# ProjectTorreyPines/TorJ.jl

Measured on AMD Instinct MI355X. Metric: ray-steps/sec, 1e5-ray EC fan on 1 MI355X (+ 2/4/8-GPU scaling), higher is better.
Workload: dtype f64

## Files before the change

### include/torj_hip.h

```cpp
#ifndef TORJ_HIP_H
#define TORJ_HIP_H

#include <stdint.h>

#ifdef __cplusplus
extern "C" {
#endif

#define TORJ_ABI_VERSION 8

enum torj_status {
    TORJ_RAY_OK = 0,
    TORJ_RAY_LEFT_PLASMA = 1,
    TORJ_RAY_ABSORBED = 2,
    TORJ_RAY_NAN = 3,
    TORJ_RAY_REFLECTED = 4,
    TORJ_RAY_ENTRY_FAIL = 5,
    TORJ_RAY_MAX_STEPS = 6
};

typedef struct torj_plasma_s *torj_plasma_t;

int torj_abi_version(void);
const char *torj_build_id(void);
// ... 224 lines not shown
                    int *steps, double *dP_shell, double *P_dep, double *traj, int n_gpus,
                    int n_shards);

typedef struct {
    int n;
    const double *x0, *N0;
    const double *weights;
    const double *psi_grid;
    const double *x_launch, *s0;
    double *state;
    int *status, *steps;
    double *dP_shell;
    double *P_dep;
    double *traj;
    uint64_t *counters;
} torj_beam_shard;
int torj_trace_beam_device(torj_plasma_t p, const torj_trace_cfg *cfg, int n_gpus, int n_psi,
                           const torj_beam_shard *shards);

int torj_set_sched(torj_plasma_t p, int mode, int waves);

int torj_trace_check(torj_plasma_t p, void *stream);

int torj_timing(torj_plasma_t p, int enable);
int torj_timing_read(torj_plasma_t p, int *calls, double *trace_ms, double *post_ms);

int torj_beam_timing_read(torj_plasma_t p, int n_gpus, int *calls, double *trace_ms, double *post_ms,
                          double *reduce_ms);

int torj_beam_comm_info(torj_plasma_t p, int n_gpus, int *device, int *nranks, int *rank);

int torj_power_deposition_profile(torj_plasma_t p, int n_rays, const int *n_points, const double *s,
                                  const double *x, const double *dP_ds, int n_psi,
                                  const double *psi_dP_dV, double *dP_dV, double *P);

int torj_shell_volumes(torj_plasma_t p, int n_psi, const double *psi_grid, double *dV);

#ifdef __cplusplus
}
#endif
#endif
```

### torj.jl_amd/csrc/torj_fitdepo.hpp

```cpp
#pragma once
#include "torj_math.hpp"

namespace torj {

constexpr int kSmpBlk = 64;
TORJ_HD size_t smp_at(size_t j, int i, size_t rows) {
    return ((size_t)((unsigned)i / kSmpBlk) * rows + j) * kSmpBlk + (unsigned)i % kSmpBlk;
}
TORJ_HD size_t smp_elems(size_t n, size_t rows) { return (n + kSmpBlk - 1) / kSmpBlk * kSmpBlk * rows; }

struct FitArgs {
    const double *coef;
    Grid g;
    int n, n_psi;
    double ds;
    const double *grid;
    const double *w;
    const double *x_launch;
    const double *s0;
    const int *steps;
    const double *smp_psi, *smp_dpds, *smp_s;
    size_t rows;
    int s_uniform;
    double *E, *Gpsi, *GP;
    int *cnt;
    double *Fopen;
    double *dPs;
    int *kstar;
    double *dP;
    double *Pray;
    const int *npts;
};

TORJ_HD int imin(int x, int y) { return x < y ? x : y; }
TORJ_HD int imax(int x, int y) { return x > y ? x : y; }

constexpr int kChunk = 8;
constexpr int kWalkChunk = 4;
constexpr int kWalkChunkStream = 1;

struct RayData {
    const FitArgs *a;
    int i, m;
    double s0, psiL;
    TORJ_HD double S(int j) const {
        if (a->npts) return a->smp_s[smp_at(j, i, a->rows)];
        if (j == 0) return 0.0;
        return a->s_uniform ? fma((double)(j - 1), a->ds, s0) : a->smp_s[smp_at(j - 1, i, a->rows)];
    }
    TORJ_HD double h(int j) const { return (j == 0 && !a->npts) ? s0 : S(j + 1) - S(j); }
    TORJ_HD double Ypsi(int j) const {
        if (a->npts) return a->smp_psi[smp_at(j, i, a->rows)];
        return j == 0 ? psiL : a->smp_psi[smp_at(j - 1, i, a->rows)];
    }
// ... 145 lines not shown
    bool spilled;
    int run_k0, run_k1, run_d;
    int runs, last_d;
    TORJ_HD void init() {
#pragma unroll
        for (int u = 0; u < NC; u++) oq[u] = -1, oF[u] = 0.0;
        spilled = false;
        run_d = 0, run_k0 = run_k1 = 0;
        runs = 0, last_d = 0;
    }
    TORJ_HD void piece(int d) {
        if (d != last_d) runs++, last_d = d;
    }
    TORJ_HD void cadd(int k, int v) {
        __hip_atomic_fetch_add(a->cnt + (size_t)k * a->n + i, v, __ATOMIC_RELAXED, __HIP_MEMORY_SCOPE_AGENT);
    }
    TORJ_HD void flush_run() {
        if (run_d == 0) return;
        const int lo = run_k0 < run_k1 ? run_k0 : run_k1, hi = run_k0 < run_k1 ? run_k1 : run_k0;
        cadd(lo, 1);
        cadd(hi + 1, -1);
        run_d = 0;
    }
    TORJ_HD void close(int q, double d) {
        double *p = a->dPs + (size_t)q * a->n + i;
        __hip_atomic_fetch_add(p, d, __ATOMIC_RELAXED, __HIP_MEMORY_SCOPE_AGENT);
    }
    TORJ_HD void toggle(int q, double Fr) {
        bool hit = false;
        double fo = 0.0;
#pragma unroll
        for (int u = 0; u < NC; u++)
            if (!hit && oq[u] == q) hit = true, fo = oF[u], oq[u] = -1;
        if (!hit && spilled) {
            double &m = a->Fopen[(size_t)q * a->n + i];
            fo = m;
            if (!isnan(fo)) hit = true, m = NAN;
        }
        if (hit) {
            close(q, fabs(Fr - fo));
            return;
        }
        bool placed = false;
#pragma unroll
        for (int u = 0; u < NC; u++)
            if (!placed && oq[u] < 0) placed = true, oq[u] = q, oF[u] = Fr;
        if (!placed) {
            a->Fopen[(size_t)oq[0] * a->n + i] = oF[0];
            spilled = true;
            oq[0] = q, oF[0] = Fr;
        }
    }
    TORJ_HD void root(int k, double Fr, int d) {
        if constexpr (CAP) {
            int &c = a->cnt[(size_t)k * a->n + i];
            if (c >= kMaxRoots) return;
            c++;
        } else if (d == run_d && k == run_k1 + d) {
            run_k1 = k;
        } else {
            flush_run();
            run_d = d, run_k0 = run_k1 = k;
        }
        if (k - 1 >= 0 && k - 1 <= a->n_psi - 2) toggle(k - 1, Fr);
        if (k <= a->n_psi - 2) toggle(k, Fr);
    }
};

template <class W_>
TORJ_HD void walk_segment(W_ &W, const Cubic &qs, double y1, const Cubic &qP, bool first) {
    const FitArgs &a = *W.a;
    const double A = 3.0 * qs.d, B = 2.0 * qs.c, C = qs.b;
    const double disc = B * B - 4.0 * A * C;
    double c1 = qs.h, c2 = qs.h;
    const double dh = fma(fma(A, qs.h, B), qs.h, C);
    const double tv = -B * A;
    const bool keep = (C > 0.0 && dh > 0.0) || (C < 0.0 && dh < 0.0);
    const bool vout = A == 0.0 || tv <= 0.0 || tv >= 2.0 * A * A * qs.h;
    if (!(keep && vout) && (A != 0.0 ? disc > 0.0 : B != 0.0)) {
        double r1 = NAN, r2 = NAN;
        if (A != 0.0) {
            const double sq = sqrt(disc);
            const double qq = -0.5 * (B + (B >= 0.0 ? sq : -sq));
            r1 = qq / A;
            if (qq != 0.0) r2 = C / qq;
        } else {
            r1 = -C / B;
        }
// ... 177 lines not shown
}

template <int NC>
TORJ_HD void fit_depo_ray(const FitArgs &a, int i, double psiL) {
    const int m = a.npts ? a.npts[i] : a.steps[i] + 2;
    if (m < 4 || (!a.npts && !(a.s0[i] > 0.0))) {
        a.kstar[i] = a.n_psi;
        a.Pray[i] = 0.0;
        return;
    }
    RayData R{&a, i, m, a.npts ? 0.0 : a.s0[i], psiL};
    nak_eliminate(R);
    Walker<NC> W{&a, i, 0.0, 0.0, Cursor{&a, 0, 0.0, 0.0}};
    W.init();
    walk_ray(W, R);
    fit_depo_finish(a, i, R, W);
}

#ifndef TORJ_DEPO_Q
#define TORJ_DEPO_Q 64
#endif
constexpr int kDepoQ = TORJ_DEPO_Q, kDepoW = 32;
enum { kDsFhi, kDsFlo, kDsOF0, kDsOF1, kDsMl, kDsMr, kDsMn, kDsMPl, kDsMPr, kDsMPn, kDsYl, kDsPl, kDsNd };
enum { kDsJ, kDsC, kDsOQ0, kDsOQ1, kDsSpill, kDsRk0, kDsRk1, kDsRd, kDsRuns, kDsLast, kDsNi };
struct DepoStream {
    double *d;
    int *v;
};
static_assert(kOpenCache == 2, "DepoStream holds two open-shell slots");

TORJ_HD bool depo_load(const DepoStream &ds, size_t n, int i, Walker<kOpenCache> &W, WalkCarry &C) {
    const int j = ds.v[kDsJ * n + i];
    if (j < 0) return false;
    const double *d = ds.d + i;
    const int *v = ds.v + i;
    W.Fhi = d[kDsFhi * n], W.Flo = d[kDsFlo * n];
    W.oF[0] = d[kDsOF0 * n], W.oF[1] = d[kDsOF1 * n];
    C.Ml = d[kDsMl * n], C.Mr = d[kDsMr * n], C.Mn = d[kDsMn * n];
    C.MPl = d[kDsMPl * n], C.MPr = d[kDsMPr * n], C.MPn = d[kDsMPn * n];
    C.yl = d[kDsYl * n], C.Pl = d[kDsPl * n];
    C.j = j;
    W.cur.c = v[kDsC * n];
    W.cur.load();
    W.oq[0] = v[kDsOQ0 * n], W.oq[1] = v[kDsOQ1 * n];
    W.spilled = v[kDsSpill * n] != 0;
    W.run_k0 = v[kDsRk0 * n], W.run_k1 = v[kDsRk1 * n], W.run_d = v[kDsRd * n];
    W.runs = v[kDsRuns * n], W.last_d = v[kDsLast * n];
    return true;
}
TORJ_HD void depo_save(const DepoStream &ds, size_t n, int i, const Walker<kOpenCache> &W, const WalkCarry &C) {
    double *d = ds.d + i;
    int *v = ds.v + i;
    d[kDsFhi * n] = W.Fhi, d[kDsFlo * n] = W.Flo;
    d[kDsOF0 * n] = W.oF[0], d[kDsOF1 * n] = W.oF[1];
    d[kDsMl * n] = C.Ml, d[kDsMr * n] = C.Mr, d[kDsMn * n] = C.Mn;
    d[kDsMPl * n] = C.MPl, d[kDsMPr * n] = C.MPr, d[kDsMPn * n] = C.MPn;
    d[kDsYl * n] = C.yl, d[kDsPl * n] = C.Pl;
    v[kDsC * n] = W.cur.c;
    v[kDsOQ0 * n] = W.oq[0], v[kDsOQ1 * n] = W.oq[1];
    v[kDsSpill * n] = W.spilled ? 1 : 0;
    v[kDsRk0 * n] = W.run_k0, v[kDsRk1 * n] = W.run_k1, v[kDsRd * n] = W.run_d;
    v[kDsRuns * n] = W.runs, v[kDsLast * n] = W.last_d;
    v[kDsJ * n] = C.j;
}

TORJ_HD bool depo_windows(const RayData &R, Walker<kOpenCache> &W, WalkCarry &C, bool started, int last) {
    for (;;) {
        const int ja = started ? C.j : 0, jb = ja + kDepoQ, r0 = jb + 2 + kDepoW;
        if (r0 + 1 > last) break;
        nak_eliminate_rows(R, started ? ja + 3 : 1, r0);
        if (!started) {
            walk_start(W, R, C);
            started = true;
        }
        walk_segments(W, R, C, jb);
    }
    return started;
}

TORJ_HD void fit_depo_stream(const FitArgs &a, const DepoStream &ds, int i, double psiL, int S) {
    if (!(a.s0[i] > 0.0)) return;
    const int j = ds.v[kDsJ * (size_t)a.n + i];
    if ((j < 0 ? 0 : j) + kDepoQ + 3 + kDepoW > S) return;
    RayData R{&a, i, S + 2, a.s0[i], psiL};
    Walker<kOpenCache> W{&a, i, 0.0, 0.0, Cursor{&a, 0, 0.0, 0.0}};
    W.init();
    WalkCarry C{};
    const bool started = depo_load(ds, a.n, i, W, C);
    if (depo_windows(R, W, C, started, S)) depo_save(ds, a.n, i, W, C);
}

TORJ_HD bool depo_next_window(const DepoStream &ds, size_t n, int i, int S, int &ja, bool &started) {
    const int j = ds.v[kDsJ * n + i];
    started = j >= 0;
    ja = started ? j : 0;
    return ja + kDepoQ + 3 + kDepoW <= S;
}
TORJ_HD void fit_depo_stream_elim(const FitArgs &a, const DepoStream &ds, int i, double psiL, int S) {
    if (!(a.s0[i] > 0.0)) return;
    int ja;
    bool started;
    if (!depo_next_window(ds, a.n, i, S, ja, started)) return;
    RayData R{&a, i, S + 2, a.s0[i], psiL};
    nak_eliminate_rows(R, started ? ja + 3 : 1, ja + kDepoQ + 2 + kDepoW);
}
TORJ_HD void fit_depo_stream_walk(const FitArgs &a, const DepoStream &ds, int i, double psiL, int S) {
    if (!(a.s0[i] > 0.0)) return;
    int ja;
    bool started;
    if (!depo_next_window(ds, a.n, i, S, ja, started)) return;
    RayData R{&a, i, S + 2, a.s0[i], psiL};
    Walker<kOpenCache> W{&a, i, 0.0, 0.0, Cursor{&a, 0, 0.0, 0.0}};
    W.init();
    WalkCarry C{};
    if (started)
        depo_load(ds, a.n, i, W, C);
    else
        walk_start(W, R, C);
    walk_segments<kWalkChunkStream>(W, R, C, ja + kDepoQ);
    depo_save(ds, a.n, i, W, C);
}

TORJ_HD void fit_depo_tail(const FitArgs &a, const DepoStream &ds, int i, double psiL) {
    const int m = a.steps[i] + 2;
    if (m < 4 || !(a.s0[i] > 0.0)) {
        a.kstar[i] = a.n_psi;
        a.Pray[i] = 0.0;
        return;
    }
    RayData R{&a, i, m, a.s0[i], psiL};
    Walker<kOpenCache> W{&a, i, 0.0, 0.0, Cursor{&a, 0, 0.0, 0.0}};
    W.init();
    WalkCarry C{};
    bool started = depo_load(ds, a.n, i, W, C);
    started = depo_windows(R, W, C, started, m - 2);
    nak_eliminate_rows(R, started ? C.j + 3 : 1, m - 2);
    if (!started) walk_start(W, R, C);
// ... 6 lines not shown
```

### torj.jl_amd/csrc/torj_hip.hip

```cpp
#include <hip/hip_runtime.h>

#include <algorithm>
#include <cmath>
#include <cstring>
#include <mutex>
#include <vector>

#include "../../include/torj_hip.h"
#include "torj_math.hpp"
#include "torj_entry.hpp"
#include "torj_fitdepo.hpp"
#include "torj_warm.hpp"

using namespace torj;

#include "torj_host_util.hpp"
#include "torj_args.hpp"
#include "torj_k_fused.hpp"
#include "torj_k_traj.hpp"
#include "torj_k_alpha.hpp"
#include "torj_k_scan.hpp"
#include "torj_k_depo.hpp"
#include "torj_k_points.hpp"
#include "torj_k_beams.hpp"
// ... 573 lines not shown
        if (p->stage.h_pinned)
            (void)hipHostFree(p->stage.h);
        else
            free(p->stage.h);
    }
    for (int r = 0; r < 2; r++) {
        if (p->stage.up[r]) (void)hipEventDestroy(p->stage.up[r]);
        if (p->stage.tr[r]) (void)hipEventDestroy(p->stage.tr[r]);
        if (p->stage.dn[r]) (void)hipEventDestroy(p->stage.dn[r]);
    }
    if (p->stage.sc) (void)hipStreamDestroy(p->stage.sc);
    if (p->d_coef) (void)hipFree(p->d_coef);
    if (p->d_cellp) (void)hipFree(p->d_cellp);
    if (p->stream) (void)hipStreamDestroy(p->stream);
    if (p->ev_Nin) (void)hipEventDestroy(p->ev_Nin);
    if (p->ev_Nout) (void)hipEventDestroy(p->ev_Nout);
    if (p->ev_U) (void)hipEventDestroy(p->ev_U);
    if (p->ev_B) (void)hipEventDestroy(p->ev_B);
    if (p->cbuild.d) (void)hipFree(p->cbuild.d);
    if (p->d_psi) (void)hipFree(p->d_psi);
    if (p->sched.d) (void)hipFree(p->sched.d);
    if (p->fit.d) (void)hipFree(p->fit.d);
    if (p->d_flags) (void)hipFree(p->d_flags);
    if (p->chunk.d) (void)hipFree(p->chunk.d);
    for (hipEvent_t e : p->ev_pool) (void)hipEventDestroy(e);
    if (p->ws.d) (void)hipFree(p->ws.d);
    if (p->beams.d) (void)hipFree(p->beams.d);
    if (p->mk.d) (void)hipFree(p->mk.d);
    if (p->split.d) (void)hipFree(p->split.d);
    if (p->batch.d) (void)hipFree(p->batch.d);
    for (int q = 0; q < torj_plasma_s::kRing; q++) {
        if (p->ev_T[q]) (void)hipEventDestroy(p->ev_T[q]);
        if (p->ev_A[q]) (void)hipEventDestroy(p->ev_A[q]);
        if (p->ev_S[q]) (void)hipEventDestroy(p->ev_S[q]);
    }
    if (p->ev_J) (void)hipEventDestroy(p->ev_J);
    if (p->ev_F) (void)hipEventDestroy(p->ev_F);
    if (p->ev_D) (void)hipEventDestroy(p->ev_D);
    if (p->stream2) (void)hipStreamDestroy(p->stream2);
    if (p->streamT) (void)hipStreamDestroy(p->streamT);
    if (p->streamS) (void)hipStreamDestroy(p->streamS);
    if (p->streamD) (void)hipStreamDestroy(p->streamD);
    delete p;
    return 0;
}

// ... 947 lines not shown
    if (!out && reduce) {
        std::vector<double *> d_dP(n_gpus);
        for (int k = 0; k < n_gpus; k++) d_dP[k] = shards[k].dP_shell;
        out = beam_reduce(p, n_gpus, d_dP, n_psi, same);
    }
    (void)hipSetDevice(p->device);
    return out;
}

int torj_trace_check(torj_plasma_t p, void *stream) {
    if (!p) return fail("bad plasma handle");
    if (!p->d_flags) return 0;
    HIPCK(hipSetDevice(p->device));
    HIPCK(hipStreamSynchronize((hipStream_t)stream));
    int flags = 0;
    HIPCK(hipMemcpy(&flags, p->d_flags, sizeof(int), hipMemcpyDeviceToHost));
    if (flags) HIPCK(hipMemset(p->d_flags, 0, sizeof(int)));
    if (flags & 1) return fail("psi_dP_dV must be strictly increasing");
    if (flags & 2) return fail("work-queue watchdog fired (ready-queue stalled)");
    if (flags & 4) return fail("work queue did not retire every ray group");
    return 0;
}

}
```

### torj.jl_amd/csrc/torj_k_depo.hpp

```cpp
#pragma once
#include "torj_args.hpp"
#include "torj_fitdepo.hpp"

constexpr int kFitGridLds = 4096;

__global__ void __launch_bounds__(64, 2) k_fit_depo(FitArgs a) {
    extern __shared__ double s_grid[];
    if (a.n_psi <= kFitGridLds) {
        for (int k = threadIdx.x; k < a.n_psi; k += 64) s_grid[k] = a.grid[k];
        __syncthreads();
        a.grid = s_grid;
    }
    const int i = blockIdx.x * 64 + threadIdx.x;
    if (i >= a.n) return;
    const double xl[3] = {a.x_launch[i], a.x_launch[a.n + i], a.x_launch[2 * a.n + i]};
    fit_depo_ray<kOpenCache>(a, i, psi_at(a.coef, a.g, xl));
}
__device__ __forceinline__ bool fit_grid_lds(FitArgs &a) {
    extern __shared__ double s_grid[];
    if (a.n_psi > kFitGridLds) return false;
    for (int k = threadIdx.x; k < a.n_psi; k += 64) s_grid[k] = a.grid[k];
    __syncthreads();
    a.grid = s_grid;
    return true;
// ... 21 lines not shown
    fit_depo_stream(a, ds, i, psiL, S);
}
#ifndef TORJ_DEPO_ELIM_WAVES
#define TORJ_DEPO_ELIM_WAVES 4
#endif
__global__ void __launch_bounds__(64, TORJ_DEPO_ELIM_WAVES) k_depo_elim(FitArgs a, DepoStream ds, const int *sinfo,
                                                                        int s_cap) {
    const int i = blockIdx.x * 64 + threadIdx.x;
    int S;
    double psiL;
    if (i >= a.n || !depo_stream_gate(a, ds, sinfo, s_cap, i, S, psiL)) return;
    fit_depo_stream_elim(a, ds, i, psiL, S);
}
#ifndef TORJ_DEPO_WALK_WAVES
#define TORJ_DEPO_WALK_WAVES 3
#endif
__global__ void __launch_bounds__(64, TORJ_DEPO_WALK_WAVES) k_depo_walk(FitArgs a, DepoStream ds, const int *sinfo,
                                                                        int s_cap) {
    fit_grid_lds(a);
    const int i = blockIdx.x * 64 + threadIdx.x;
    int S;
    double psiL;
    if (i >= a.n || !depo_stream_gate(a, ds, sinfo, s_cap, i, S, psiL)) return;
    fit_depo_stream_walk(a, ds, i, psiL, S);
}
__global__ void __launch_bounds__(64, 2) k_depo_tail(FitArgs a, DepoStream ds) {
    fit_grid_lds(a);
    const int i = blockIdx.x * 64 + threadIdx.x;
    if (i >= a.n) return;
    const double xl[3] = {a.x_launch[i], a.x_launch[a.n + i], a.x_launch[2 * a.n + i]};
    fit_depo_tail(a, ds, i, psi_at(a.coef, a.g, xl));
}
__global__ void __launch_bounds__(64) k_profile_samples(FitArgs a, const long *off, const double *s,
                                                        const double *x, size_t n_all, const double *dpds) {
    const int i = blockIdx.x * 64 + threadIdx.x;
    if (i >= a.n) return;
    for (int j = 0; j < a.npts[i]; j++) {
        const size_t q = (size_t)off[i] + j;
        const double xq[3] = {x[q], x[n_all + q], x[2 * n_all + q]};
        const size_t o = smp_at(j, i, a.rows);
        const_cast<double *>(a.smp_psi)[o] = psi_at(a.coef, a.g, xq);
        const_cast<double *>(a.smp_dpds)[o] = dpds[q];
        const_cast<double *>(a.smp_s)[o] = s[q];
    }
}
__global__ void __launch_bounds__(64, 2) k_fit_profile(FitArgs a) {
    extern __shared__ double s_grid[];
// ... 48 lines not shown
```

### torj.jl_amd/csrc/torj_plasma.hpp

```cpp
#pragma once
#include <rccl/rccl.h>

#include <algorithm>
#include <mutex>
#include <vector>

#include "torj_args.hpp"
#include "torj_host_util.hpp"
#include "torj_math.hpp"

static void bspl1d_prefilter(int n, const double *y, size_t ystride, double *c, size_t cstride) {
    auto C = [&](int k) -> double & { return c[(size_t)k * cstride]; };
    auto Y = [&](int k) { return y[(size_t)k * ystride]; };
    C(1) = Y(0);
    C(n) = Y(n - 1);
    const int m = n - 2;
    if (m > 0) {
        std::vector<double> cp(m), dp(m);
        for (int k = 0; k < m; k++) {
            double r = 6.0 * Y(k + 1);
            if (k == 0) r -= C(1);
            if (k == m - 1) r -= C(n);
            const double den = 4.0 - (k > 0 ? cp[k - 1] : 0.0);
            cp[k] = 1.0 / den;
// ... 94 lines not shown
    std::vector<double> coef;
    std::vector<double> psi_nodes;
    double *d_coef = nullptr;
    double *d_cellp = nullptr;
    int n_vol = 0;
    double v1 = 0, vn = 0;
    std::vector<double> vol_coef;
    double psi_prof_max = 0;
    hipStream_t stream = nullptr;
    GrowBuf sched;
    int sched_mode = -1, sched_waves = 0;
    int lanes_per_ray = 0;
    GrowBuf chunk;
    GrowBuf fit;
    bool timing = false;
    int timing_calls = 0;
    GrowBuf batch;
    std::vector<hipEvent_t> ev_pool;
    size_t ev_used = 0;
    GrowBuf ws;
    GrowBuf beams;
    GrowBuf mk;
    int *d_flags = nullptr;
    int n_cu = 256;
    std::mutex mu;
    std::vector<torj_plasma_s *> replicas;
    std::vector<ncclComm_t> comms;
    struct BeamStage {
        void *d = nullptr, *h = nullptr;
        size_t d_cap = 0, h_cap = 0;
        bool h_pinned = false;
        hipStream_t sc = nullptr;
        hipEvent_t up[2] = {}, tr[2] = {}, dn[2] = {};
    } stage;
    double reduce_ms = 0.0;
    int reduce_calls = 0;
    GrowBuf split;
    hipStream_t stream2 = nullptr, streamT = nullptr;
    hipStream_t streamS = nullptr;
    hipStream_t streamD = nullptr;
    static constexpr int kRing = kSplitRing;
    hipEvent_t ev_T[kRing] = {}, ev_A[kRing] = {}, ev_S[kRing] = {}, ev_J = nullptr, ev_F = nullptr;
    hipEvent_t ev_D = nullptr;
    hipEvent_t ev_Nin = nullptr, ev_Nout = nullptr;
    hipEvent_t ev_U = nullptr;
    GrowBuf cbuild;
// ... 34 lines not shown
    return 0;
}

static int ensure_device(torj_plasma_s *p) {
    std::lock_guard<std::mutex> lk(p->mu);
    int ndev = 0;
    HIPCK(hipGetDeviceCount(&ndev));
    if (p->device < 0 || p->device >= ndev)
        return fail("device %d not available (%d HIP devices)", p->device, ndev);
    HIPCK(hipSetDevice(p->device));
    if (p->d_flags) return 0;
    if (p->d_coef) return fail("handle's device state is incomplete (an earlier initialisation failed)");
    HIPCK(hipMalloc(&p->d_coef, p->coef.size() * sizeof(double)));
    HIPCK(hipMemcpy(p->d_coef, p->coef.data(), p->coef.size() * sizeof(double),
                    hipMemcpyHostToDevice));
    {
        std::vector<double> cp((size_t)(p->g.nR - 1) * (p->g.nZ - 1) * kCellRec);
        cell_power_table(p->coef.data(), p->g.nR, p->g.nZ, p->g.hR, p->g.hZ, cp.data());
        HIPCK(hipMalloc(&p->d_cellp, cp.size() * sizeof(double)));
        HIPCK(hipMemcpy(p->d_cellp, cp.data(), cp.size() * sizeof(double), hipMemcpyHostToDevice));
    }
    HIPCK(hipStreamCreateWithFlags(&p->stream, hipStreamNonBlocking));
    HIPCK(hipDeviceGetAttribute(&p->n_cu, hipDeviceAttributeMultiprocessorCount, p->device));
    int *flags = nullptr;
    HIPCK(hipMalloc(&flags, sizeof(int)));
    if (hipMemset(flags, 0, sizeof(int)) != hipSuccess) {
        (void)hipFree(flags);
        return fail("hipMemset of the launch flags failed");
    }
    p->d_flags = flags;
    return 0;
}

static int ensure_buf(torj_plasma_s *p, GrowBuf &b, size_t bytes) {
    std::lock_guard<std::mutex> lk(p->mu);
    return b.reserve(bytes);
}

static int mirror_sync(torj_plasma_s *p) {
    std::lock_guard<std::mutex> lk(p->mu);
    if (!p->coef_stale && !p->psi_stale) return 0;
    HIPCK(hipSetDevice(p->device));
    HIPCK(hipEventSynchronize(p->ev_B));
    if (p->coef_stale) {
        HIPCK(hipMemcpy(p->coef.data(), p->d_coef, p->coef.size() * sizeof(double), hipMemcpyDeviceToHost));
        p->coef_stale = false;
// ... 78 lines not shown
```

### torj.jl_amd/csrc/torj_split.hpp

```cpp
#pragma once
#include <algorithm>
#include <atomic>

#include "torj_args.hpp"
#include "torj_fitdepo.hpp"
#include "torj_host_util.hpp"
#ifndef TORJ_SPLIT_PLAN_ONLY
#include "torj_dispatch.hpp"
#include "torj_k_alpha.hpp"
#include "torj_k_depo.hpp"
#include "torj_k_scan.hpp"
#include "torj_k_traj.hpp"
#include "torj_plasma.hpp"

static size_t fit_grid_lds(int n_psi) { return n_psi <= kFitGridLds ? (size_t)n_psi * sizeof(double) : 0; }

static int fit_zero(const FitArgs &fa, hipStream_t st) {
    const size_t L = (size_t)fa.n_psi, N = (size_t)fa.n;
    HIPCK(hipMemsetAsync(fa.cnt, 0, (L + 1) * N * sizeof(int), st));
    HIPCK(hipMemsetAsync(fa.Fopen, 0xFF, L * N * sizeof(double), st));
    HIPCK(hipMemsetAsync(fa.dPs, 0, L * N * sizeof(double), st));
    return 0;
}
#endif
// ... 127 lines not shown
    sp.tx = (double *)take(6 * pl.b_n8);
    sp.stau = (double *)take(pl.b_n8);
    sp.spsi = (double *)take(pl.b_n8);
    sp.sPdep = (double *)take(pl.b_n8);
    sp.tinfo = (int *)take(pl.b_n4);
    sp.sinfo = (int *)take(pl.b_n4);
    sp.defer = pl.b_defer ? (unsigned long long *)take(pl.b_defer) : nullptr;
    rg.dcnt = pl.b_dcnt ? (unsigned *)take(pl.b_dcnt) : nullptr;
    if (pl.dstream) {
        rg.ds.d = (double *)take(pl.b_dsd);
        rg.ds.v = (int *)take(pl.b_dsi);
    }
}

#ifndef TORJ_SPLIT_PLAN_ONLY
static int split_plan(SplitPlan &pl, const torj_plasma_s *p, const TraceArgs &a, int DM, bool walk,
                      bool negl_skip) {
    size_t free_b = 0, total_b = 0;
    HIPCK(hipMemGetInfo(&free_b, &total_b));
    split_plan_sizes(pl, p->sched_mode, p->sched_waves, free_b, a, DM, walk, negl_skip);
    return 0;
}

static int split_trace(torj_plasma_s *p, TraceArgs a, int DM, bool tr, hipStream_t s, const FitArgs *fa,
                       DepoStream *dso, bool negl_skip, double tiny_alpha) {
    SplitPlan pl;
    if (split_plan(pl, p, a, DM, fa && dso, negl_skip)) return -1;
    constexpr int R = SplitPlan::R;
    const size_t n = pl.n;
    if (ensure_split(p, pl.bytes)) return -1;
    SplitArgs sp{};
    SplitRing rg;
    split_carve(pl, (char *)p->split.d, sp, rg);
    const DepoStream ds = rg.ds;
    if (dso) *dso = ds;
    sp.nf = pl.nf;
    sp.tile_cap = pl.tile_cap;
    sp.tile_margin = pl.tile_margin;
    sp.nan_step = pl.nan_step;
    sp.zval = 0.0;
    sp.defer_lrm = pl.defer_lrm;
    sp.zlatch = pl.zlatch;
    sp.tiny_alpha = split_tiny_alpha(pl, a, tiny_alpha);
    sp.tval = 0.0;
    const int tflag_nan_from = env_has("TORJ_TEST_TFLAG_NAN") ? std::max(0, env_int("TORJ_TEST_TFLAG_NAN", 0)) : -1;
    if (tflag_nan_from >= 0) {
        static std::atomic<bool> warned{false};
        if (!warned.exchange(true))
            fprintf(stderr, "libtorj_hip: TORJ_TEST_TFLAG_NAN is set -- a TEST HOOK: alpha waves fully "
                            "flagged by the tiny_alpha proof write NaN\n");
    }

    const bool serial = pl.serial, dstream = pl.dstream;
    static const bool scan_own = env_int("TORJ_SPLIT_SCAN", 1) != 0;
    hipStream_t sT = serial ? s : p->streamT, s2 = serial ? s : p->stream2;
    hipStream_t s3 = serial ? s : (scan_own ? p->streamS : p->stream2);
    const bool depo_own = dstream && (pl.dstream_env == 2 || pl.dstream_env == 4) && !serial;
    const bool depo_traj = dstream && pl.dstream_env == 5 && !serial;
    if (depo_own && !p->streamD) {
        int lo = 0, hi = 0;
        HIPCK(hipDeviceGetStreamPriorityRange(&lo, &hi));
        HIPCK(hipStreamCreateWithPriority(&p->streamD, hipStreamNonBlocking, stream_prio("TORJ_DEPO_PRIO", lo, lo, hi)));
    }
    hipStream_t sD = depo_own ? p->streamD : s3;
    if (!serial) {
        HIPCK(hipEventRecord(p->ev_F, s));
        HIPCK(hipStreamWaitEvent(sT, p->ev_F, 0));
        HIPCK(hipStreamWaitEvent(s2, p->ev_F, 0));
        if (s3 != s2) HIPCK(hipStreamWaitEvent(s3, p->ev_F, 0));
    }
    HIPCK(hipMemsetAsync(sp.stau, 0, 3 * pl.b_n8, sT));
    HIPCK(hipMemsetAsync(sp.sinfo, 0, pl.b_n4, sT));
    if (dstream) HIPCK(hipMemsetAsync(ds.v + kDsJ * n, 0xFF, n * sizeof(int), sT));
    if (rg.dcnt) HIPCK(hipMemsetAsync(rg.dcnt, 0, pl.n_blk * sizeof(unsigned), s2));
    if (fa && fit_zero(*fa, s3)) return -1;
    const size_t fit_lds = fa ? fit_grid_lds(fa->n_psi) : 0;
    const int G = (int)((n + 63) / 64);
    const size_t lds_bytes = pl.traj_lds_bytes;
    const bool lds_traj = pl.traj_mode == kTrajLds;
    const bool tile_traj = pl.traj_mode == kTrajTile, cell_traj = pl.traj_mode == kTrajCell;
    sp.traj_mode = pl.traj_mode;
    const int wpb = std::min(8, std::max(1, (G + p->n_cu - 1) / p->n_cu));
    const int n_blocks = pl.n_blk;
    auto depo_pair = [&](hipStream_t st, int cap) {
        hipLaunchKernelGGL(k_depo_elim, dim3(G), dim3(64), 0, st, *fa, ds, sp.sinfo, cap);
        hipLaunchKernelGGL(k_depo_walk, dim3(G), dim3(64), fit_lds, st, *fa, ds, sp.sinfo, cap);
    };
    for (int b = 0; b < n_blocks; b++) {
        sp.k0 = pl.block_k0(b);
        sp.kb = pl.block_len(b);
        const int r = b % R;
        sp.ain = rg.ain[r];
        sp.psib = rg.psib[r];
        sp.zflag = rg.zflags[r];
        sp.gflag = rg.gflags[r];
        sp.zval = (pl.zflag_nan_from >= 0 && sp.k0 >= pl.zflag_nan_from) ? NAN : 0.0;
        sp.tval = (tflag_nan_from >= 0 && sp.k0 >= tflag_nan_from) ? NAN : 0.0;
        sp.alpha = rg.alphas[r];
        sp.awork = pl.b_awork ? rg.aworks[r] : nullptr;
        if (b >= R) HIPCK(hipStreamWaitEvent(sT, p->ev_S[r], 0));
        if (depo_traj && b >= pl.depo_lag) {
            const int bw = b - pl.depo_lag;
            HIPCK(hipStreamWaitEvent(sT, p->ev_S[bw % R], 0));
            depo_pair(sT, pl.window_cap(bw));
        }
        with_depo_traj(DM, tr, [&](auto D, auto T) {
            if (cell_traj)
                hipLaunchKernelGGL((k_traj_cell<D(), T()>), dim3(G), dim3(64), 0, sT, a, sp);
            else if (tile_traj)
// ... 81 lines not shown
```

### torj.jl_amd/torj_hip/_lib.py

```python
from __future__ import annotations

import ctypes as C
import os
import subprocess

import numpy as np

_PKG = os.path.dirname(os.path.abspath(__file__))
_ROOT = os.path.dirname(_PKG)
LIB_PATH = os.environ.get("TORJ_HIP_LIB") or os.path.join(_ROOT, "build", "libtorj_hip.so")
CSRC = os.path.join(_ROOT, "csrc")

_dp = C.POINTER(C.c_double)
_ip = C.POINTER(C.c_int)
_u64p = C.POINTER(C.c_uint64)
_hp = C.POINTER(C.c_void_p)


class TorjError(RuntimeError):
    pass


class TraceCfg(C.Structure):
    _fields_ = [("omega", C.c_double), ("mode", C.c_int), ("ds", C.c_double),
# ... 69 lines not shown
    "torj_abs_albajar_fast": (C.c_int, [C.c_int, _dp, _dp, _dp, _dp, _dp, _dp, C.c_int, _dp]),
    "torj_alpha_warm": (C.c_int, [C.c_int] + [_dp] * 7 + [C.c_int, C.c_int, _dp, _dp]),
    "torj_refractive_index_sq": (C.c_int, [C.c_int, _dp, _dp, _dp, C.c_int, _dp]),
    "torj_pol_tor_angles_2_vector": (None, [C.c_double, C.c_double, _dp]),
    "torj_launch_peripheral_rays": (C.c_int, [_dp, _dp, C.c_double, C.c_double, C.c_double,
                                              C.c_int, C.c_int, C.c_int, _ip, _dp, _dp, _dp]),
    "torj_ray_entry": (C.c_int, [C.c_void_p, C.c_int, _dp, _dp, C.c_double, C.c_int, _dp, _dp,
                                 _dp, _ip]),
    "torj_ray_entry_device": (C.c_int, [C.c_void_p, C.c_int, C.c_void_p, C.c_void_p, C.c_double,
                                        C.c_int, C.c_void_p, C.c_void_p, C.c_void_p, C.c_void_p,
                                        C.c_void_p]),
    "torj_ray_entry_gpu": (C.c_int, [C.c_void_p, C.c_int, _dp, _dp, C.c_double, C.c_int, _dp,
                                     _dp, _dp, _ip]),
    "torj_trace": (C.c_int, [C.c_void_p, C.POINTER(TraceCfg), C.c_int, _dp, _dp, _dp, C.c_int,
                             _dp, _dp, _ip, _ip, _dp, _dp, _dp]),
    "torj_trace_ex": (C.c_int, [C.c_void_p, C.POINTER(TraceCfg), C.c_int, _dp, _dp, _dp, C.c_int,
                                _dp, _dp, _dp, _dp, _ip, _ip, _dp, _dp, _dp]),
    "torj_trace_beam": (C.c_int, [C.c_void_p, C.POINTER(TraceCfg), C.c_int, _dp, _dp, _dp, C.c_int,
                                  _dp, _dp, _dp, _dp, _ip, _ip, _dp, _dp, _dp, C.c_int, C.c_int]),
    "torj_trace_beam_device": (C.c_int, [C.c_void_p, C.POINTER(TraceCfg), C.c_int, C.c_int,
                                         C.POINTER(BeamShard)]),
    "torj_set_sched": (C.c_int, [C.c_void_p, C.c_int, C.c_int]),
    "torj_trace_check": (C.c_int, [C.c_void_p, C.c_void_p]),
    "torj_timing": (C.c_int, [C.c_void_p, C.c_int]),
    "torj_timing_read": (C.c_int, [C.c_void_p, _ip, _dp, _dp]),
    "torj_beam_timing_read": (C.c_int, [C.c_void_p, C.c_int, _ip, _dp, _dp, _dp]),
    "torj_beam_comm_info": (C.c_int, [C.c_void_p, C.c_int, _ip, _ip, _ip]),
    "torj_trace_device": (C.c_int, [C.c_void_p, C.POINTER(TraceCfg), C.c_int, C.c_void_p,
                                    C.c_void_p, C.c_void_p, C.c_int, C.c_void_p, C.c_void_p,
                                    C.c_void_p, C.c_void_p, C.c_void_p, C.c_void_p, C.c_void_p,
                                    C.c_void_p, C.c_void_p]),
    "torj_trace_device_ex": (C.c_int, [C.c_void_p, C.POINTER(TraceCfg), C.c_int] +
                             [C.c_void_p] * 3 + [C.c_int] + [C.c_void_p] * 11),
    "torj_trace_beams_device": (C.c_int, [C.c_void_p, C.POINTER(TraceCfg), C.c_int, _ip, _dp, _ip] +
                                [C.c_void_p] * 3 + [C.c_int] + [C.c_void_p] * 11),
    "torj_trace_beams": (C.c_int, [C.c_void_p, C.POINTER(TraceCfg), C.c_int, _ip, _dp, _ip, _dp, _dp,
                                   _dp, C.c_int, _dp, _dp, _dp, _dp, _ip, _ip, _dp, _dp, _dp]),
    "torj_ray_entry_beams_device": (C.c_int, [C.c_void_p, C.c_int, _ip, _dp, _ip] + [C.c_void_p] * 7),
    "torj_ray_entry_beams_gpu": (C.c_int, [C.c_void_p, C.c_int, _ip, _dp, _ip, _dp, _dp, _dp, _dp, _dp,
                                           _ip]),
    "torj_trace_beams_plasmas_device": (C.c_int, [C.c_void_p, C.c_int, _hp, _ip, C.POINTER(TraceCfg), C.c_int,
                                                  _ip, _dp, _ip] + [C.c_void_p] * 3 + [C.c_int] +
                                        [C.c_void_p] * 11),
    "torj_trace_beams_plasmas": (C.c_int, [C.c_void_p, C.c_int, _hp, _ip, C.POINTER(TraceCfg), C.c_int, _ip, _dp,
                                           _ip, _dp, _dp, _dp, C.c_int, _dp, _dp, _dp, _dp, _ip, _ip, _dp, _dp,
                                           _dp]),
# ... 74 lines not shown
```

### torj.jl_amd/torj_hip/plasma.py

```python
from __future__ import annotations

import ctypes as C

import numpy as np

from ._lib import check, dptr, f64, lib, soa

FIELDS = ("psi", "lnne", "lnTe", "Br", "Bz", "Bphi")


class Plasma:

    def __init__(self, R_coords, Z_coords, psi_norm_data, psi_prof, ne_prof, Te_prof, Br_data,
                 Bz_data, Bphi_data, eqt1d_psi_norm, eqt1d_volume, device: int = 0):
        R, Z = f64(R_coords), f64(Z_coords)
        nR, nZ = len(R), len(Z)

        def m(a):
            a = np.asarray(a, dtype=np.float64)
            if a.shape != (nR, nZ):
                raise ValueError(f"2-D map has shape {a.shape}, expected {(nR, nZ)}")
            return np.ascontiguousarray(a.T)

        keep = [m(psi_norm_data), f64(psi_prof), f64(ne_prof), f64(Te_prof), m(Br_data),
# ... 127 lines not shown
    def __del__(self):
        h = getattr(self, "_h", None)
        if h is not None and h.value:
            try:
                lib().torj_plasma_destroy(h)
            except Exception:
                pass
            self._h = None

    def coefs(self, field: str) -> np.ndarray:
        nR, nZ = len(self.R_coords), len(self.Z_coords)
        out = np.zeros((nZ + 2) * (nR + 2))
        check(lib().torj_plasma_get_coefs(self._h, FIELDS.index(field), dptr(out)))
        return out.reshape(nZ + 2, nR + 2).T.copy()

    def volume(self, psi):
        p = np.atleast_1d(f64(psi))
        out = np.zeros_like(p)
        check(lib().torj_plasma_volume(self._h, len(p), dptr(p), dptr(out)))
        return out if np.ndim(psi) else float(out[0])

    def set_sched(self, mode: int = -1, waves: int = 0):
        check(lib().torj_set_sched(self._h, int(mode), int(waves)))

    def shell_volumes(self, psi_grid):
        g = f64(psi_grid)
        dV = np.zeros(max(len(g) - 1, 0))
        check(lib().torj_shell_volumes(self._h, len(g), dptr(g), dptr(dV)))
        return dV

    def eval_points(self, x, N=None, omega: float = 1.0) -> np.ndarray:
        xs = soa(x)
        n = xs.shape[1]
        Ns = soa(N) if N is not None else np.zeros_like(xs)
        out = np.zeros((13, n))
        check(lib().torj_eval_plasma(self._h, n, dptr(xs), dptr(Ns), omega, dptr(out)))
        return out


def _single(x):
    return np.asarray(x).ndim == 1


def evaluate(plasma: Plasma, field: str, x):
    if field not in ("psi", "psi_norm_spline"):
        raise ValueError("only the psi_norm spline is exposed point-wise; use n_e/T_e/B_spline")
# ... 47 lines not shown
```

Baseline: 6.392 billion.

## Add powerless fast path for deposition windows with zero absorbed power

Adds a fast path to the windowed deposition fit that first checks whether every ray in a wavefront has zero power samples and zero carried power state in the current window. When that holds, it eliminates only the psi spline system and walks segments with constant F, skipping zero-valued atomic adds. The streaming walk is split into two kernels (a regular path and a new powerless kernel) chosen per wave. A device counter and API are added to report how many windows took the fast path. The cost is an extra kernel launch, per-window stat atomics, and a more complex control flow with wave-uniform gating.

Result: slower. 6.075 billion (-5.0%).

```diff
diff --git a/include/torj_hip.h b/include/torj_hip.h
--- a/include/torj_hip.h
+++ b/include/torj_hip.h
@@ -270,6 +270,8 @@
 
 int torj_trace_check(torj_plasma_t p, void *stream);
 
+int torj_depo_window_stats(torj_plasma_t p, void *stream, unsigned long long *fast, unsigned long long *total);
+
 int torj_timing(torj_plasma_t p, int enable);
 int torj_timing_read(torj_plasma_t p, int *calls, double *trace_ms, double *post_ms);
 
diff --git a/torj.jl_amd/csrc/torj_fitdepo.hpp b/torj.jl_amd/csrc/torj_fitdepo.hpp
--- a/torj.jl_amd/csrc/torj_fitdepo.hpp
+++ b/torj.jl_amd/csrc/torj_fitdepo.hpp
@@ -1,4 +1,6 @@
 #pragma once
+#include <stdlib.h>
+
 #include "torj_math.hpp"
 
 namespace torj {
@@ -30,6 +32,8 @@
     double *dP;
     double *Pray;
     const int *npts;
+    int zfast;
+    unsigned long long *zstat;
 };
 
 TORJ_HD int imin(int x, int y) { return x < y ? x : y; }
@@ -221,11 +225,12 @@
         cadd(hi + 1, -1);
         run_d = 0;
     }
-    TORJ_HD void close(int q, double d) {
+    TORJ_HD void close(int q, double d, bool skip0 = false) {
+        if (skip0 && d == 0.0) return;
         double *p = a->dPs + (size_t)q * a->n + i;
         __hip_atomic_fetch_add(p, d, __ATOMIC_RELAXED, __HIP_MEMORY_SCOPE_AGENT);
     }
-    TORJ_HD void toggle(int q, double Fr) {
+    TORJ_HD void toggle(int q, double Fr, bool skip0 = false) {
         bool hit = false;
         double fo = 0.0;
 #pragma unroll
@@ -237,7 +242,7 @@
             if (!isnan(fo)) hit = true, m = NAN;
         }
         if (hit) {
-            close(q, fabs(Fr - fo));
+            close(q, fabs(Fr - fo), skip0);
             return;
         }
         bool placed = false;
@@ -250,7 +255,7 @@
             oq[0] = q, oF[0] = Fr;
         }
     }
-    TORJ_HD void root(int k, double Fr, int d) {
+    TORJ_HD void root(int k, double Fr, int d, bool skip0 = false) {
         if constexpr (CAP) {
             int &c = a->cnt[(size_t)k * a->n + i];
             if (c >= kMaxRoots) return;
@@ -261,8 +266,8 @@
             flush_run();
             run_d = d, run_k0 = run_k1 = k;
         }
-        if (k - 1 >= 0 && k - 1 <= a->n_psi - 2) toggle(k - 1, Fr);
-        if (k <= a->n_psi - 2) toggle(k, Fr);
+        if (k - 1 >= 0 && k - 1 <= a->n_psi - 2) toggle(k - 1, Fr, skip0);
+        if (k <= a->n_psi - 2) toggle(k, Fr, skip0);
     }
 };
 
@@ -486,7 +491,7 @@
 #endif
 constexpr int kDepoQ = TORJ_DEPO_Q, kDepoW = 32;
 enum { kDsFhi, kDsFlo, kDsOF0, kDsOF1, kDsMl, kDsMr, kDsMn, kDsMPl, kDsMPr, kDsMPn, kDsYl, kDsPl, kDsNd };
-enum { kDsJ, kDsC, kDsOQ0, kDsOQ1, kDsSpill, kDsRk0, kDsRk1, kDsRd, kDsRuns, kDsLast, kDsNi };
+enum { kDsJ, kDsZ, kDsC, kDsOQ0, kDsOQ1, kDsSpill, kDsRk0, kDsRk1, kDsRd, kDsRuns, kDsLast, kDsNi };
 struct DepoStream {
     double *d;
     int *v;
@@ -528,17 +533,248 @@
     v[kDsJ * n] = C.j;
 }
 
-TORJ_HD bool depo_windows(const RayData &R, Walker<kOpenCache> &W, WalkCarry &C, bool started, int last) {
+TORJ_HD void depo_save_powerless(const DepoStream &ds, size_t n, int i, const Walker<kOpenCache> &W,
+                                 const WalkCarry &C, bool started) {
+    double *d = ds.d + i;
+    int *v = ds.v + i;
+    if (!started) d[kDsFhi * n] = 0.0, d[kDsFlo * n] = 0.0;
+    d[kDsOF0 * n] = W.oF[0], d[kDsOF1 * n] = W.oF[1];
+    d[kDsMl * n] = C.Ml, d[kDsMr * n] = C.Mr, d[kDsMn * n] = C.Mn;
+    d[kDsMPl * n] = 0.0, d[kDsMPr * n] = 0.0, d[kDsMPn * n] = 0.0;
+    d[kDsYl * n] = C.yl, d[kDsPl * n] = 0.0;
+    v[kDsC * n] = W.cur.c;
+    v[kDsOQ0 * n] = W.oq[0], v[kDsOQ1 * n] = W.oq[1];
+    v[kDsSpill * n] = W.spilled ? 1 : 0;
+    v[kDsRk0 * n] = W.run_k0, v[kDsRk1 * n] = W.run_k1, v[kDsRd * n] = W.run_d;
+    v[kDsRuns * n] = W.runs, v[kDsLast * n] = W.last_d;
+    v[kDsJ * n] = C.j;
+}
+
+static_assert((kDepoQ + kDepoW) % kChunk == 0, "a later window's elimination reads whole chunks: no sample below its rows");
+#ifndef __HIP_DEVICE_COMPILE__
+inline unsigned long long g_depo_zfast = 0, g_depo_windows = 0;
+#endif
+TORJ_HD bool depo_zfast_on(const FitArgs &a) {
+#ifdef __HIP_DEVICE_COMPILE__
+    return a.zfast != 0;
+#else
+    (void)a;
+    const char *e = getenv("TORJ_DEPO_ZFAST");
+    return !e || atoi(e) != 0;
+#endif
+}
+TORJ_HD bool wave_all(bool p) {
+#ifdef __HIP_DEVICE_COMPILE__
+    return __all(p);
+#else
+    return p;
+#endif
+}
+TORJ_HD void depo_count(const FitArgs &a, bool fast) {
+#ifdef __HIP_DEVICE_COMPILE__
+    if (!a.zstat) return;
+    const unsigned long long act = __ballot(1);
+    if ((int)__lane_id() == __ffsll((long long)act) - 1)
+        __hip_atomic_fetch_add(a.zstat + (fast ? 0 : 1), (unsigned long long)__popcll(act), __ATOMIC_RELAXED,
+                               __HIP_MEMORY_SCOPE_AGENT);
+#else
+    (void)a;
+    (fast ? g_depo_zfast : g_depo_windows)++;
+#endif
+}
+TORJ_HD unsigned long long dbits(double x) { return __builtin_bit_cast(unsigned long long, x); }
+
+TORJ_HD bool nak_eliminate_rows_psi(const RayData &R, int r_lo, int r_hi) {
+    const int m = R.m;
+    const double h0 = R.h(0), h1 = R.h(1);
+    double yn = R.Ypsi(r_hi + 1), yc = R.Ypsi(r_hi);
+    unsigned long long nz = dbits(R.YP(r_hi + 1)) | dbits(R.YP(r_hi)) | dbits(R.YP(imax(r_lo - 2, 0)));
+    double hr = R.h(r_hi), ihr = rcp_nz(hr);
+    double e = 0.0, gp = 0.0;
+    for (int r0 = r_hi; r0 >= r_lo; r0 -= kChunk) {
+        double yv[kChunk];
+#pragma unroll
+        for (int u = 0; u < kChunk; u++) {
+            const int j = imax(r0 - 1 - u, 0);
+            yv[u] = R.Ypsi(j);
+            nz |= dbits(R.YP(j));
+        }
+        if (!wave_all((nz << 1) == 0)) return false;
+#pragma unroll
+        for (int u = 0; u < kChunk; u++) {
+            const int r = r0 - u;
+            if (r < r_lo) break;
+            const double hl = R.h(r - 1), ihl = rcp_nz(hl);
+            const double yl = yv[u];
+            const double rp = 6.0 * ((yn - yc) * ihr - (yc - yl) * ihl);
+            double sub = hl, dia = 2.0 * (hl + hr), sup = hr;
+            if (r == 1) {
+                dia = 3.0 * h0 + 2.0 * h1 + h0 * h0 / h1;
+                sup = h1 - h0 * h0 / h1;
+                sub = 0.0;
+            }
+            if (r == m - 2) {
+                const double hm2 = hr, hm3 = hl;
+                sub = hm3 - hm2 * hm2 / hm3;
+                dia = 2.0 * hm3 + 3.0 * hm2 + hm2 * hm2 / hm3;
+                sup = 0.0;
+            }
+            const double iden = rcp_nz(dia - sup * e);
+            gp = (rp - sup * gp) * iden;
+            e = sub * iden;
+            R.EE(r) = e;
+            R.GPSI(r) = gp;
+            yn = yc, yc = yl, hr = hl, ihr = ihl;
+        }
+    }
+    return true;
+}
+TORJ_HD bool carry_powerless(double MPl, double MPr, double MPn, double Pl, double Fhi, double Flo) {
+    return ((dbits(MPl) | dbits(MPr) | dbits(MPn) | dbits(Pl)) << 1) == 0 && fabs(Fhi) < INFINITY &&
+           fabs(Flo) < INFINITY;
+}
+TORJ_HD bool depo_eliminate(const RayData &R, int r_lo, int r_hi, bool zc) {
+    const bool z = nak_eliminate_rows_psi(R, r_lo, r_hi);
+    const bool fast = wave_all(z && zc);
+    if (!z) {
+        nak_eliminate_rows(R, r_lo, r_hi);
+    } else if (!fast) {
+        for (int r = r_hi; r >= r_lo; r--) R.GPP(r) = 0.0;
+    } else if (r_lo == 1) {
+        R.GPP(1) = 0.0, R.GPP(2) = 0.0;
+    }
+    return fast;
+}
+
+template <class W_>
+TORJ_HD void walk_segment_powerless(W_ &W, const Cubic &qs, double y1, double F, bool first) {
+    const FitArgs &a = *W.a;
+    const double A = 3.0 * qs.d, B = 2.0 * qs.c, C = qs.b;
+    const double disc = B * B - 4.0 * A * C;
+    double c1 = qs.h, c2 = qs.h;
+    const double dh = fma(fma(A, qs.h, B), qs.h, C);
+    const double tv = -B * A;
+    const bool keep = (C > 0.0 && dh > 0.0) || (C < 0.0 && dh < 0.0);
+    const bool vout = A == 0.0 || tv <= 0.0 || tv >= 2.0 * A * A * qs.h;
+    if (!(keep && vout) && (A != 0.0 ? disc > 0.0 : B != 0.0)) {
+        double r1 = NAN, r2 = NAN;
+        if (A != 0.0) {
+            const double sq = sqrt(disc);
+            const double qq = -0.5 * (B + (B >= 0.0 ? sq : -sq));
+            r1 = qq / A;
+            if (qq != 0.0) r2 = C / qq;
+        } else {
+            r1 = -C / B;
+        }
+        if (r2 < r1) {
+            const double t = r1;
+            r1 = r2;
+            r2 = t;
+        }
+        const bool in1 = r1 > 0.0 && r1 < qs.h, in2 = r2 > 0.0 && r2 < qs.h && r2 != r1;
+        if (in1) c1 = r1;
+        if (in2) {
+            if (in1)
+                c2 = r2;
+            else
+                c1 = r2;
+        }
+    }
+    double fa = qs.y0, ta = 0.0;
+#pragma unroll 1
+    for (int p = 0; p < 3; p++) {
+        const double tb = p == 0 ? c1 : (p == 1 ? c2 : qs.h);
+        if (!(tb > ta) && p > 0) continue;
+        const double fb = (tb == qs.h) ? y1 : qs.f(tb);
+        const bool first0 = first && p == 0;
+        int k, kend, d;
+        if (fb > fa) {
+            d = 1;
+            W.piece(1);
+            k = first0 ? level_above(a, fa, false) : W.cur.c;
+            W.cur.seek(fb);
+            kend = W.cur.c;
+        } else if (fb < fa) {
+            d = -1;
+            W.piece(-1);
+            k = (first0 ? level_above(a, fa, true) : W.cur.c - (fa == W.cur.lo)) - 1;
+            W.cur.seek(fb);
+            kend = W.cur.c - (fb == W.cur.lo) - 1;
+        } else {
+            W.cur.seek(fb);
+            d = 0, k = kend = 0;
+        }
+        for (; d > 0 ? k < kend : k > kend; k += d) W.root(k, F, d, true);
+        fa = fb, ta = tb;
+        if (tb == qs.h) break;
+    }
+}
+
+template <int WC = kWalkChunk, class W_>
+TORJ_HD void walk_segments_powerless(W_ &W, const RayData &R, WalkCarry &C, int j_end) {
+    const int m = R.m;
+    double Ml = C.Ml, Mr = C.Mr, Mn = C.Mn, yl = C.yl;
+    const double F = W.Fhi + W.Flo;
+    for (int j0 = C.j; j0 < j_end; j0 += WC) {
+        double yv[WC], ev[WC], gv[WC];
+#pragma unroll
+        for (int u = 0; u < WC; u++) {
+            yv[u] = R.Ypsi(imin(j0 + 1 + u, m - 1));
+            const int r = imin(j0 + 3 + u, m - 2);
+            ev[u] = R.EE(r);
+            gv[u] = R.GPSI(r);
+        }
+#pragma unroll
+        for (int u = 0; u < WC; u++) {
+            const int j = j0 + u;
+            if (j >= j_end) break;
+            const double h = R.h(j), ih = rcp_nz(h);
+            walk_segment_powerless(W, make_cubic(yl, yv[u], Ml, Mr, h, ih), yv[u], F, j == 0);
+            yl = yv[u];
+            Ml = Mr, Mr = Mn;
+            if (j + 3 <= m - 2) {
+                Mn = gv[u] - ev[u] * Mr;
+            } else if (j + 3 == m - 1) {
+                const double q1 = R.h(m - 2) / R.h(m - 3);
+                Mn = (1.0 + q1) * Mr - q1 * Ml;
+            }
+        }
+    }
+    C.Ml = Ml, C.Mr = Mr, C.Mn = Mn, C.MPl = 0.0, C.MPr = 0.0, C.MPn = 0.0;
+    C.yl = yl, C.Pl = 0.0;
+    C.j = j_end;
+}
+
+__host__ __device__ __attribute__((noinline)) inline bool depo_windows_call(const RayData &R, Walker<kOpenCache> &W,
+                                                                            WalkCarry &C, bool started, int last) {
+    const bool zon = depo_zfast_on(*R.a);
     for (;;) {
         const int ja = started ? C.j : 0, jb = ja + kDepoQ, r0 = jb + 2 + kDepoW;
         if (r0 + 1 > last) break;
-        nak_eliminate_rows(R, started ? ja + 3 : 1, r0);
-        if (!started) {
-            walk_start(W, R, C);
-            started = true;
-        }
-        walk_segments(W, R, C, jb);
-    }
+        const int r_lo = started ? ja + 3 : 1;
+        bool fast = false;
+        if (zon) {
+            const bool zc = !started || carry_powerless(C.MPl, C.MPr, C.MPn, C.Pl, W.Fhi, W.Flo);
+            fast = depo_eliminate(R, r_lo, r0, zc);
+            depo_count(*R.a, fast);
+        } else {
+            nak_eliminate_rows(R, r_lo, r0);
+        }
+        if (!started) walk_start(W, R, C);
+        started = true;
+        if (fast)
+            walk_segments_powerless(W, R, C, jb);
+        else
+            walk_segments(W, R, C, jb);
+    }
+    return started;
+}
+TORJ_HD bool depo_windows(const RayData &R, Walker<kOpenCache> &W, WalkCarry &C, bool started, int last) {
+    const RayData Rt = R;
+    Walker<kOpenCache> Wt = W;
+    WalkCarry Ct = C;
+    started = depo_windows_call(Rt, Wt, Ct, started, last);
+    W = Wt, C = Ct;
     return started;
 }
 
@@ -566,8 +802,20 @@
     bool started;
     if (!depo_next_window(ds, a.n, i, S, ja, started)) return;
     RayData R{&a, i, S + 2, a.s0[i], psiL};
-    nak_eliminate_rows(R, started ? ja + 3 : 1, ja + kDepoQ + 2 + kDepoW);
-}
+    const int r_lo = started ? ja + 3 : 1, r_hi = ja + kDepoQ + 2 + kDepoW;
+    if (!depo_zfast_on(a)) {
+        nak_eliminate_rows(R, r_lo, r_hi);
+        return;
+    }
+    bool zc = true;
+    if (started) {
+        const double *d = ds.d + i;
+        const size_t n = a.n;
+        zc = carry_powerless(d[kDsMPl * n], d[kDsMPr * n], d[kDsMPn * n], d[kDsPl * n], d[kDsFhi * n], d[kDsFlo * n]);
+    }
+    ds.v[kDsZ * (size_t)a.n + i] = depo_eliminate(R, r_lo, r_hi, zc) ? ja + 1 : 0;
+}
+template <int PART = 0>
 TORJ_HD void fit_depo_stream_walk(const FitArgs &a, const DepoStream &ds, int i, double psiL, int S) {
     if (!(a.s0[i] > 0.0)) return;
     int ja;
@@ -577,6 +825,24 @@
     Walker<kOpenCache> W{&a, i, 0.0, 0.0, Cursor{&a, 0, 0.0, 0.0}};
     W.init();
     WalkCarry C{};
+    bool fast = false;
+    if (depo_zfast_on(a)) {
+        fast = wave_all(ds.v[kDsZ * (size_t)a.n + i] == ja + 1);
+        if (PART != (fast ? 1 : 2)) depo_count(a, fast);
+    }
+    if (PART == (fast ? 1 : 2)) return;
+    if (fast) {
+        if constexpr (PART != 1) {
+            if (started)
+                depo_load(ds, a.n, i, W, C);
+            else
+                walk_start(W, R, C);
+            walk_segments_powerless<kWalkChunkStream>(W, R, C, ja + kDepoQ);
+            depo_save_powerless(ds, a.n, i, W, C, started);
+        }
+        return;
+    }
+    if constexpr (PART == 2) return;
     if (started)
         depo_load(ds, a.n, i, W, C);
     else
diff --git a/torj.jl_amd/csrc/torj_hip.hip b/torj.jl_amd/csrc/torj_hip.hip
--- a/torj.jl_amd/csrc/torj_hip.hip
+++ b/torj.jl_amd/csrc/torj_hip.hip
@@ -619,6 +619,7 @@
     if (p->sched.d) (void)hipFree(p->sched.d);
     if (p->fit.d) (void)hipFree(p->fit.d);
     if (p->d_flags) (void)hipFree(p->d_flags);
+    if (p->d_zstat) (void)hipFree(p->d_zstat);
     if (p->chunk.d) (void)hipFree(p->chunk.d);
     for (hipEvent_t e : p->ev_pool) (void)hipEventDestroy(e);
     if (p->ws.d) (void)hipFree(p->ws.d);
@@ -1612,4 +1613,18 @@
     return 0;
 }
 
-}
+int torj_depo_window_stats(torj_plasma_t p, void *stream, unsigned long long *fast, unsigned long long *total) {
+    if (!p) return fail("bad plasma handle");
+    unsigned long long z[2] = {0, 0};
+    if (p->d_zstat) {
+        HIPCK(hipSetDevice(p->device));
+        HIPCK(hipStreamSynchronize((hipStream_t)stream));
+        HIPCK(hipMemcpy(z, p->d_zstat, sizeof(z), hipMemcpyDeviceToHost));
+        if (z[0] | z[1]) HIPCK(hipMemset(p->d_zstat, 0, sizeof(z)));
+    }
+    if (fast) *fast = z[0];
+    if (total) *total = z[0] + z[1];
+    return 0;
+}
+
+}
diff --git a/torj.jl_amd/csrc/torj_k_depo.hpp b/torj.jl_amd/csrc/torj_k_depo.hpp
--- a/torj.jl_amd/csrc/torj_k_depo.hpp
+++ b/torj.jl_amd/csrc/torj_k_depo.hpp
@@ -67,7 +67,19 @@
     int S;
     double psiL;
     if (i >= a.n || !depo_stream_gate(a, ds, sinfo, s_cap, i, S, psiL)) return;
-    fit_depo_stream_walk(a, ds, i, psiL, S);
+    fit_depo_stream_walk<1>(a, ds, i, psiL, S);
+}
+#ifndef TORJ_DEPO_WALKZ_WAVES
+#define TORJ_DEPO_WALKZ_WAVES 3
+#endif
+__global__ void __launch_bounds__(64, TORJ_DEPO_WALKZ_WAVES) k_depo_walk_z(FitArgs a, DepoStream ds, const int *sinfo,
+                                                                           int s_cap) {
+    fit_grid_lds(a);
+    const int i = blockIdx.x * 64 + threadIdx.x;
+    int S;
+    double psiL;
+    if (i >= a.n || !depo_stream_gate(a, ds, sinfo, s_cap, i, S, psiL)) return;
+    fit_depo_stream_walk<2>(a, ds, i, psiL, S);
 }
 __global__ void __launch_bounds__(64, 2) k_depo_tail(FitArgs a, DepoStream ds) {
     fit_grid_lds(a);
diff --git a/torj.jl_amd/csrc/torj_plasma.hpp b/torj.jl_amd/csrc/torj_plasma.hpp
--- a/torj.jl_amd/csrc/torj_plasma.hpp
+++ b/torj.jl_amd/csrc/torj_plasma.hpp
@@ -140,6 +140,7 @@
     GrowBuf beams;
     GrowBuf mk;
     int *d_flags = nullptr;
+    unsigned long long *d_zstat = nullptr;
     int n_cu = 256;
     std::mutex mu;
     std::vector<torj_plasma_s *> replicas;
@@ -220,6 +221,10 @@
     }
     HIPCK(hipStreamCreateWithFlags(&p->stream, hipStreamNonBlocking));
     HIPCK(hipDeviceGetAttribute(&p->n_cu, hipDeviceAttributeMultiprocessorCount, p->device));
+    if (!p->d_zstat) {
+        HIPCK(hipMalloc(&p->d_zstat, 2 * sizeof(unsigned long long)));
+        HIPCK(hipMemset(p->d_zstat, 0, 2 * sizeof(unsigned long long)));
+    }
     int *flags = nullptr;
     HIPCK(hipMalloc(&flags, sizeof(int)));
     if (hipMemset(flags, 0, sizeof(int)) != hipSuccess) {
diff --git a/torj.jl_amd/csrc/torj_split.hpp b/torj.jl_amd/csrc/torj_split.hpp
--- a/torj.jl_amd/csrc/torj_split.hpp
+++ b/torj.jl_amd/csrc/torj_split.hpp
@@ -173,10 +173,11 @@
     return 0;
 }
 
-static int split_trace(torj_plasma_s *p, TraceArgs a, int DM, bool tr, hipStream_t s, const FitArgs *fa,
+static int split_trace(torj_plasma_s *p, TraceArgs a, int DM, bool tr, hipStream_t s, FitArgs *fa,
                        DepoStream *dso, bool negl_skip, double tiny_alpha) {
     SplitPlan pl;
     if (split_plan(pl, p, a, DM, fa && dso, negl_skip)) return -1;
+    if (fa) fa->zfast = env_int("TORJ_DEPO_ZFAST", 1) != 0, fa->zstat = p->d_zstat;
     constexpr int R = SplitPlan::R;
     const size_t n = pl.n;
     if (ensure_split(p, pl.bytes)) return -1;
@@ -222,7 +223,8 @@
     }
     HIPCK(hipMemsetAsync(sp.stau, 0, 3 * pl.b_n8, sT));
     HIPCK(hipMemsetAsync(sp.sinfo, 0, pl.b_n4, sT));
-    if (dstream) HIPCK(hipMemsetAsync(ds.v + kDsJ * n, 0xFF, n * sizeof(int), sT));
+    static_assert(kDsZ == kDsJ + 1, "one clear for both rows");
+    if (dstream) HIPCK(hipMemsetAsync(ds.v + kDsJ * n, 0xFF, 2 * n * sizeof(int), sT));
     if (rg.dcnt) HIPCK(hipMemsetAsync(rg.dcnt, 0, pl.n_blk * sizeof(unsigned), s2));
     if (fa && fit_zero(*fa, s3)) return -1;
     const size_t fit_lds = fa ? fit_grid_lds(fa->n_psi) : 0;
@@ -236,6 +238,7 @@
     auto depo_pair = [&](hipStream_t st, int cap) {
         hipLaunchKernelGGL(k_depo_elim, dim3(G), dim3(64), 0, st, *fa, ds, sp.sinfo, cap);
         hipLaunchKernelGGL(k_depo_walk, dim3(G), dim3(64), fit_lds, st, *fa, ds, sp.sinfo, cap);
+        if (fa->zfast) hipLaunchKernelGGL(k_depo_walk_z, dim3(G), dim3(64), fit_lds, st, *fa, ds, sp.sinfo, cap);
     };
     for (int b = 0; b < n_blocks; b++) {
         sp.k0 = pl.block_k0(b);
diff --git a/torj.jl_amd/torj_hip/_lib.py b/torj.jl_amd/torj_hip/_lib.py
--- a/torj.jl_amd/torj_hip/_lib.py
+++ b/torj.jl_amd/torj_hip/_lib.py
@@ -115,6 +115,7 @@
                                          C.POINTER(BeamShard)]),
     "torj_set_sched": (C.c_int, [C.c_void_p, C.c_int, C.c_int]),
     "torj_trace_check": (C.c_int, [C.c_void_p, C.c_void_p]),
+    "torj_depo_window_stats": (C.c_int, [C.c_void_p, C.c_void_p, _u64p, _u64p]),
     "torj_timing": (C.c_int, [C.c_void_p, C.c_int]),
     "torj_timing_read": (C.c_int, [C.c_void_p, _ip, _dp, _dp]),
     "torj_beam_timing_read": (C.c_int, [C.c_void_p, C.c_int, _ip, _dp, _dp, _dp]),
diff --git a/torj.jl_amd/torj_hip/plasma.py b/torj.jl_amd/torj_hip/plasma.py
--- a/torj.jl_amd/torj_hip/plasma.py
+++ b/torj.jl_amd/torj_hip/plasma.py
@@ -173,6 +173,11 @@
 
     def set_sched(self, mode: int = -1, waves: int = 0):
         check(lib().torj_set_sched(self._h, int(mode), int(waves)))
+
+    def depo_window_stats(self, stream=None):
+        fast, total = C.c_uint64(0), C.c_uint64(0)
+        check(lib().torj_depo_window_stats(self._h, stream, C.byref(fast), C.byref(total)))
+        return int(fast.value), int(total.value)
 
     def shell_volumes(self, psi_grid):
         g = f64(psi_grid)
```
